# zjykzj/YOLOv4

Hardware: AMD Instinct MI355X
Metric: images/sec fwd+bwd @608x608 bs=64 per GPU (YOLOv4 training step: forward + YOLOLoss + backward) (higher is better)
Workload: dtype f32

## Files before the change

yolov4_amd/csrc/conv_planes.hip:

```cpp
#include <stdlib.h>
#include <type_traits>
#include "common.h"
#include "conv_geom.h"

namespace {

typedef _Float16 f16x8 __attribute__((ext_vector_type(8)));
typedef float f32x4v __attribute__((ext_vector_type(4)));

__device__ __host__ __forceinline__ unsigned pl_scale_exp(unsigned amax_bits) {
    const unsigned e = (amax_bits >> 23) & 0xffu;
    if (e == 0u || e == 255u) return 127u;
    int se = 268 - (int)e;
    if (se < 2) se = 2;
    if (se > 252) se = 252;
    return (unsigned)se;
}
__device__ __forceinline__ float pl_scale(const unsigned* amax) { return __uint_as_float(pl_scale_exp(amax ? *amax : 0u) << 23); }
__device__ __forceinline__ float pl_unscale(const unsigned* amax) { return __uint_as_float((254u - pl_scale_exp(amax ? *amax : 0u)) << 23); }

struct PlaneConvGeom {
    const unsigned char* src;
    const unsigned char* wt;
    float* dst; long long ldd;
    const float* res; long long ldr;
    float* stats;
    int dst_bf16;
    int cls_ntaps, cls_ph, cls_pw, Hfull, Wfull;
    int cls_dh[4], cls_dw[4], cls_slot[4];
    int B, Hs, Ws, Cs, Hd, Wd, N, k, stride, pad, M, K;
    int mtiles, ntiles;
    unsigned long long src_total_bytes;
    unsigned wt_bytes;
    const unsigned* src_amax; const unsigned* wt_amax;
};

constexpr int PROW = 128;

typedef __bf16 bf16x8 __attribute__((ext_vector_type(8)));
template <bool BF>
__device__ __forceinline__ f32x4v pl_mma(const f16x8 a, const f16x8 b, const f32x4v c) {
    if constexpr (BF) return __builtin_amdgcn_mfma_f32_16x16x32_bf16(__builtin_bit_cast(bf16x8, a), __builtin_bit_cast(bf16x8, b), c, 0, 0, 0);
    else return __builtin_amdgcn_mfma_f32_16x16x32_f16(a, b, c, 0, 0, 0);
}

#ifndef PL_ST_POL
#define PL_ST_POL 2
#endif
template <int BM, int BN, int WM, int WN, bool BF, bool YB = false, bool DG2 = false>
__global__ __launch_bounds__(WM * WN * 64, WM * WN == 8 ? 1 : 2) void conv_planes_mfma(const PlaneConvGeom g) {
    constexpr int NWAVE = WM * WN, NTHR = NWAVE * 64;
    static_assert(NWAVE == 8 || NWAVE == 4, "8 or 4 waves");
    constexpr int WTM = BM / WM, WTN = BN / WN, TM = WTM / 16, TN = WTN / 16;
    constexpr int A_BYTES = BM * PROW, B_BYTES = BN * PROW, STAGE = A_BYTES + B_BYTES;
    constexpr int NSTAGE = (NWAVE == 8 && 3 * STAGE <= 160 * 1024) ? 3 : 2;
    constexpr int KSH = BF ? 6 : 5;
    constexpr unsigned WEB = BF ? 2u : 4u;
    constexpr int PA = BM / 8 / NWAVE, PB = BN / 8 / NWAVE, NDMA = PA + PB;
    static_assert(PA >= 1 && PB >= 1 && ((NSTAGE == 3 && NDMA == 6) || (NSTAGE == 2 && NDMA == 8)),
                  "the counted vmcnt below assumes 6 (three stages) or 8 (two stages) pieces per wave and K-tile");
    typedef float accv __attribute__((ext_vector_type(4)));
    extern __shared__ __attribute__((aligned(1024))) unsigned char smem[];

    const int tid = threadIdx.x, lane = tid & 63;
    const int wave = __builtin_amdgcn_readfirstlane(tid >> 6);
    const int wm = wave / WN, wn = wave % WN;
    const int lt = y4_xcd_remap(blockIdx.x, g.mtiles * g.ntiles);
    const int mt = lt / g.ntiles, nt = lt - mt * g.ntiles;
    const int n0 = nt * BN;
    const int CC = g.Cs >> KSH;
    const int KT = (DG2 ? g.cls_ntaps : g.k * g.k) * CC;

    const int pix_per_img = g.Hd * g.Wd;
    const int b_first = (int)(((long long)mt * BM) / pix_per_img);
    const unsigned pitch = (unsigned)g.Cs * 4u;
    const unsigned long long img_bytes = (unsigned long long)g.Hs * g.Ws * pitch;
    const unsigned long long skip = (unsigned long long)b_first * img_bytes;
    const unsigned long long left = g.src_total_bytes > skip ? g.src_total_bytes - skip : 0ull;
    const __amdgpu_buffer_rsrc_t src_rsrc = y4_make_rsrc(g.src + skip, (unsigned)(left < 0xfffffff0ull ? left : 0xfffffff0ull));
    const __amdgpu_buffer_rsrc_t wt_rsrc = y4_make_rsrc(g.wt, g.wt_bytes);
    const unsigned OOB = 0xffffffffu;

    const int lr = lane >> 3, pos = lane & 7;
    unsigned a_base[PA], a_valid[PA], a_voff[PA];
#pragma unroll
    for (int i = 0; i < PA; ++i) {
        const int row = (wave * PA + i) * 8 + lr;
        const int m = mt * BM + row;
        const bool ok = m < g.M;
        const int mm = ok ? m : 0;
        const int b = mm / pix_per_img;
        const int rem = mm - b * pix_per_img;
        const int hd = rem / g.Wd, wd = rem - hd * g.Wd;
        const int hc = DG2 ? hd : hd * g.stride - g.pad, wc = DG2 ? wd : wd * g.stride - g.pad;
        const int chunk = pos ^ ((row >> 1) & 7);
        a_base[i] = (unsigned)(((b - b_first) * g.Hs + hc) * g.Ws + wc) * pitch + (unsigned)chunk * 16u;
        unsigned v = 0u;
        if constexpr (DG2) {
            for (int t = 0; t < g.cls_ntaps; ++t)
                if (ok && hc + g.cls_dh[t] < g.Hs && wc + g.cls_dw[t] < g.Ws) v |= 1u << t;
        } else {
            for (int r = 0; r < g.k; ++r)
                for (int q = 0; q < g.k; ++q)
                    if (ok && (unsigned)(hc + r) < (unsigned)g.Hs && (unsigned)(wc + q) < (unsigned)g.Ws) v |= 1u << (r * g.k + q);
        }
        a_valid[i] = v;
    }
    unsigned b_off[PB];
#pragma unroll
    for (int j = 0; j < PB; ++j) {
        const int row = (wave * PB + j) * 8 + lr;
        const int chunk = pos ^ ((row >> 1) & 7);
        b_off[j] = (n0 + row) < g.N ? (unsigned)(n0 + row) * (unsigned)g.K * WEB + (unsigned)chunk * 16u : OOB;
    }
    int ld_tap = 0, ld_r = 0, ld_q = 0, ld_cc = 0;
    int ld_slot = DG2 ? g.cls_slot[0] : 0;
    auto tap_setup = [&]() {
        unsigned toff;
        if constexpr (DG2) {
            const int t = ld_tap < g.cls_ntaps ? ld_tap : 0;
            toff = (unsigned)(g.cls_dh[t] * g.Ws + g.cls_dw[t]) * pitch;
            ld_slot = g.cls_slot[t];
        } else {
            toff = (unsigned)(ld_r * g.Ws + ld_q) * pitch;
            ld_slot = ld_tap;
        }
#pragma unroll
        for (int i = 0; i < PA; ++i) a_voff[i] = ((a_valid[i] >> ld_tap) & 1u) ? a_base[i] + toff : OOB;
    };
    tap_setup();
    typedef __attribute__((address_space(3))) void* lds_ptr;
    auto issue = [&](int stage, auto P0, auto P1) {
        constexpr int p0 = decltype(P0)::value, p1 = decltype(P1)::value;
        unsigned char* st = smem + stage * STAGE;
        const unsigned soff_a = (unsigned)ld_cc * 128u;
        const unsigned soff_b = (unsigned)(ld_slot * CC + ld_cc) * 128u;
#pragma unroll
        for (int p = p0; p < p1; ++p) {
            if (p < PA)
                __builtin_amdgcn_raw_ptr_buffer_load_lds(src_rsrc, (lds_ptr)(st + (wave * PA + p) * 1024), 16, (int)a_voff[p], (int)soff_a, 0, 0);
            else
                __builtin_amdgcn_raw_ptr_buffer_load_lds(wt_rsrc, (lds_ptr)(st + A_BYTES + (wave * PB + (p - PA)) * 1024), 16,
                                                         (int)b_off[p - PA], (int)soff_b, 0, 0);
        }
        if constexpr (p1 == NDMA) {
            if (++ld_cc == CC) {
                ld_cc = 0; ++ld_tap;
                if (++ld_q == g.k) { ld_q = 0; ++ld_r; }
                tap_setup();
            }
        }
    };
    using I0 = std::integral_constant<int, 0>; using I2 = std::integral_constant<int, 2>; using I4 = std::integral_constant<int, 4>;
    using I6 = std::integral_constant<int, NDMA>;

    accv acc0[TM][TN], acc1[BF ? 1 : TM][BF ? 1 : TN];
#pragma unroll
    for (int i = 0; i < TM; ++i)
#pragma unroll
        for (int j = 0; j < TN; ++j)
#pragma unroll
            for (int e = 0; e < 4; ++e) {
                acc0[i][j][e] = 0.f;
                if constexpr (!BF) acc1[i][j][e] = 0.f;
            }

    const int fr = lane & 15, kq = lane >> 4;
    const int sw = (fr >> 1) & 7;
    const int a_hi = (wm * WTM + fr) * PROW + ((kq ^ sw) << 4), a_lo = (wm * WTM + fr) * PROW + (((4 + kq) ^ sw) << 4);
    const int b_hi = A_BYTES + (wn * WTN + fr) * PROW + ((kq ^ sw) << 4), b_lo = A_BYTES + (wn * WTN + fr) * PROW + (((4 + kq) ^ sw) << 4);

    bool pend = false;
    auto step = [&](auto SC, const int kt) {
        constexpr int S = decltype(SC)::value;
        const unsigned char* base = smem + S * STAGE;
        f16x8 fb[TN][2];
#pragma unroll
        for (int j = 0; j < TN; ++j) {
            fb[j][0] = *reinterpret_cast<const f16x8*>(base + b_hi + j * 16 * PROW);
            fb[j][1] = *reinterpret_cast<const f16x8*>(base + b_lo + j * 16 * PROW);
        }
        f16x8 fap[2][2];
        fap[0][0] = *reinterpret_cast<const f16x8*>(base + a_hi);
        fap[0][1] = *reinterpret_cast<const f16x8*>(base + a_lo);
#pragma unroll
        for (int i = 0; i < TM; ++i) {
            if (i + 1 < TM) {
                fap[(i + 1) & 1][0] = *reinterpret_cast<const f16x8*>(base + a_hi + (i + 1) * 16 * PROW);
                fap[(i + 1) & 1][1] = *reinterpret_cast<const f16x8*>(base + a_lo + (i + 1) * 16 * PROW);
            }
            const f16x8 fa0 = fap[i & 1][0], fa1 = fap[i & 1][1];
            if (i == TM - 1) {
                __builtin_amdgcn_sched_barrier(0);
                asm volatile("s_waitcnt lgkmcnt(0)" ::: "memory");
                if (kt + 1 < KT) {
                    if constexpr (NSTAGE == 3) {
                        if (kt + 2 < KT) asm volatile("s_waitcnt vmcnt(6)" ::: "memory");
                        else asm volatile("s_waitcnt vmcnt(0)" ::: "memory");
                        __builtin_amdgcn_s_barrier();
                        if (kt + 3 < KT) { issue(S, I0{}, I2{}); pend = true; }
                    } else {
                        asm volatile("s_waitcnt vmcnt(0)" ::: "memory");
                        __builtin_amdgcn_s_barrier();
                        if (kt + 2 < KT) issue(S, I0{}, I6{});
                    }
                }
            }
            if constexpr (BF) {
#pragma unroll
                for (int j = 0; j < TN; ++j) acc0[i][j] = pl_mma<true>(fa0, fb[j][0], acc0[i][j]);
#pragma unroll
                for (int j = 0; j < TN; ++j) acc0[i][j] = pl_mma<true>(fa1, fb[j][1], acc0[i][j]);
            } else {
#pragma unroll
                for (int j = 0; j < TN; ++j) {
                    acc1[i][j] = pl_mma<false>(fa1, fb[j][0], acc1[i][j]);
                    acc1[i][j] = pl_mma<false>(fa0, fb[j][1], acc1[i][j]);
                    acc0[i][j] = pl_mma<false>(fa0, fb[j][0], acc0[i][j]);
                }
            }
            if constexpr (NSTAGE == 3) {
                if (i == 0 && pend) issue((S + 2) % NSTAGE, I2{}, I4{});
                if (i == 1 && pend) { issue((S + 2) % NSTAGE, I4{}, I6{}); pend = false; }
            }
        }
    };
    static_assert(TM >= 3, "the DMA pieces are spread over the first three row tiles");

    for (int t = 0; t < NSTAGE && t < KT; ++t) issue(t, I0{}, I6{});
    if constexpr (NSTAGE == 3) {
        if (KT >= 3) asm volatile("s_waitcnt vmcnt(12)" ::: "memory");
        else if (KT == 2) asm volatile("s_waitcnt vmcnt(6)" ::: "memory");
        else asm volatile("s_waitcnt vmcnt(0)" ::: "memory");
    } else {
        if (KT >= 2) asm volatile("s_waitcnt vmcnt(8)" ::: "memory");
        else asm volatile("s_waitcnt vmcnt(0)" ::: "memory");
    }
    __builtin_amdgcn_s_barrier();
    if constexpr (NSTAGE == 3) {
        int kt = 0;
        for (; kt + 3 <= KT; kt += 3) {
            step(std::integral_constant<int, 0>{}, kt);
            step(std::integral_constant<int, 1>{}, kt + 1);
            step(std::integral_constant<int, 2>{}, kt + 2);
        }
        if (kt < KT) step(std::integral_constant<int, 0>{}, kt);
        if (kt + 1 < KT) step(std::integral_constant<int, 1>{}, kt + 1);
    } else {
        int kt = 0;
        for (; kt + 2 <= KT; kt += 2) {
            step(std::integral_constant<int, 0>{}, kt);
            step(std::integral_constant<int, 1>{}, kt + 1);
        }
        if (kt < KT) step(std::integral_constant<int, 0>{}, kt);
    }

    const float un = BF ? 1.0f : pl_unscale(g.src_amax) * pl_unscale(g.wt_amax);
    const float un1 = un * (1.0f / 2048.0f);
    auto result = [&](int i, int j, int e) -> float {
        if constexpr (BF) return acc0[i][j][e];
        else return acc0[i][j][e] * un + acc1[i][j][e] * un1;
    };
    {
        const unsigned drow = (unsigned)g.ldd * 4u, rrow = (unsigned)g.ldr * 4u;
        const long long row0 = (long long)mt * BM;
        const unsigned long long left = (unsigned long long)(g.M - row0);
        const unsigned long long dby = left * drow, rby = g.ldr ? left * rrow : (unsigned long long)g.N * 4ull;
        const __amdgpu_buffer_rsrc_t drs = y4_make_rsrc(reinterpret_cast<char*>(g.dst) + row0 * (long long)drow, (unsigned)(dby < 0xfffffff0ull ? dby : 0xfffffff0ull));
        const __amdgpu_buffer_rsrc_t rrs = y4_make_rsrc(g.res ? reinterpret_cast<const char*>(g.res) + row0 * (long long)rrow : nullptr,
                                                        g.res ? (unsigned)(rby < 0xfffffff0ull ? rby : 0xfffffff0ull) : 0u);
        int lane_e = lane;
        asm volatile("" : "+v"(lane_e));
        const int fr = lane_e & 15, kq = lane_e >> 4;
        const int colb = n0 + wn * WTN + fr;
        const bool allc = n0 + BN <= g.N;
        if constexpr (DG2) {
            const __amdgpu_buffer_rsrc_t xrs = y4_make_rsrc(g.dst, (unsigned)((unsigned long long)g.B * g.Hfull * g.Wfull * drow));
#pragma unroll
            for (int i = 0; i < TM; ++i) {
                const int m0 = mt * BM + wm * WTM + 16 * i + 4 * kq;
                int b = m0 / pix_per_img;
                const int rem = m0 - b * pix_per_img;
                int hc = rem / g.Wd, wc = rem - hc * g.Wd;
#pragma unroll
                for (int e = 0; e < 4; ++e) {
                    const bool rok = m0 + e < g.M;
                    const unsigned po = (unsigned)((b * g.Hfull + 2 * hc + g.cls_ph) * g.Wfull + 2 * wc + g.cls_pw) * drow + (unsigned)colb * 4u;
#pragma unroll
                    for (int j = 0; j < TN; ++j) {
// ... 46 lines not shown
                        const bool cok = allc || colb + 16 * j < g.N;
                        __builtin_amdgcn_raw_buffer_store_b32(__builtin_bit_cast(unsigned, v), drs, (int)(cok ? dvo + 64u * j : 0xffffffffu), (int)(e * drow), PL_ST_POL);
                    }
            }
        }
        } else {
            float csum[TN], cssum[TN];
#pragma unroll
            for (int j = 0; j < TN; ++j) { csum[j] = 0.f; cssum[j] = 0.f; }
#pragma unroll
            for (int i = 0; i < TM; ++i) {
                const unsigned rl = (unsigned)(wm * WTM + 16 * i + 4 * kq);
                const unsigned dvo = rl * drow + (unsigned)colb * 2u;
#pragma unroll
                for (int e = 0; e < 4; ++e)
#pragma unroll
                    for (int j = 0; j < TN; ++j) {
                        const float v = result(i, j, e);
                        unsigned u = __builtin_bit_cast(unsigned, v);
                        u = (u + 0x7fffu + ((u >> 16) & 1u)) & 0xffff0000u;
                        const float vr = __builtin_bit_cast(float, u);
                        csum[j] += vr; cssum[j] += vr * vr;
                        const unsigned nb = (unsigned)__builtin_amdgcn_update_dpp(0, (int)u, 0xB1, 0xf, 0xf, true);
                        const bool cok = (allc || colb + 16 * j < g.N) && !(fr & 1);
                        __builtin_amdgcn_raw_buffer_store_b32((u >> 16) | nb, drs, (int)(cok ? dvo + 32u * j : 0xffffffffu), (int)(e * drow), PL_ST_POL);
                    }
                __builtin_amdgcn_sched_barrier(0);
            }
#pragma unroll
            for (int j = 0; j < TN; ++j) { acc0[0][j][0] = csum[j]; acc0[0][j][1] = cssum[j]; }
        }
    }
    if (g.stats) {
        __syncthreads();
        float* red = reinterpret_cast<float*>(smem);
#pragma unroll
        for (int j = 0; j < TN; ++j) {
            float cs = 0.f, css = 0.f;
            if constexpr (YB) {
                cs = acc0[0][j][0]; css = acc0[0][j][1];
            } else {
#pragma unroll
                for (int i = 0; i < TM; ++i)
#pragma unroll
                    for (int e = 0; e < 4; ++e) { const float v = acc0[i][j][e]; cs += v; css += v * v; }
            }
            cs += __shfl_xor(cs, 16, 64); css += __shfl_xor(css, 16, 64);
            cs += __shfl_xor(cs, 32, 64); css += __shfl_xor(css, 32, 64);
            if (kq == 0) {
                const int c = wn * WTN + j * 16 + fr;
                red[(wm * BN + c) * 2 + 0] = cs;
                red[(wm * BN + c) * 2 + 1] = css;
            }
        }
        __syncthreads();
        for (int c = tid; c < BN; c += NTHR) {
            float cs = 0.f, css = 0.f;
#pragma unroll
            for (int w = 0; w < WM; ++w) { cs += red[(w * BN + c) * 2]; css += red[(w * BN + c) * 2 + 1]; }
            const int n = n0 + c;
            if (n < g.N) {
                g.stats[((long long)mt * 2 + 0) * g.N + n] = cs;
                g.stats[((long long)mt * 2 + 1) * g.N + n] = css;
            }
        }
    }
}

struct PlaneWgradGeom {
    const unsigned char* x;
    const unsigned char* dy;
    float* out;
    int B, H, W, Cin, Cout, k, pad, M, J;
    int ldy_ch;
    int ntn, ntj, splits, steps_per_split;
    unsigned long long x_total_bytes, dy_total_bytes;
    const unsigned* x_amax; const unsigned* dy_amax;
};

typedef __fp16 trh4 __attribute__((__vector_size__(4 * sizeof(__fp16))));
__device__ __forceinline__ f16x8 tr_frag(const unsigned char* p) {
    typedef __attribute__((address_space(3))) trh4* lp;
    const trh4 a = __builtin_amdgcn_ds_read_tr16_b64_v4f16((lp)(p));
    const trh4 b = __builtin_amdgcn_ds_read_tr16_b64_v4f16((lp)(p + 4 * PROW));
    f16x8 r;
#pragma unroll
    for (int e = 0; e < 4; ++e) { r[e] = (_Float16)a[e]; r[4 + e] = (_Float16)b[e]; }
    return r;
}

template <int N> __device__ __forceinline__ void pl_wait_vm() {
    static_assert(N == 0 || N == 3 || N == 4 || N == 6 || N == 8 || N == 12, "add the literal");
    if constexpr (N == 0) asm volatile("s_waitcnt vmcnt(0)" ::: "memory");
    else if constexpr (N == 3) asm volatile("s_waitcnt vmcnt(3)" ::: "memory");
    else if constexpr (N == 4) asm volatile("s_waitcnt vmcnt(4)" ::: "memory");
    else if constexpr (N == 6) asm volatile("s_waitcnt vmcnt(6)" ::: "memory");
    else if constexpr (N == 8) asm volatile("s_waitcnt vmcnt(8)" ::: "memory");
    else asm volatile("s_waitcnt vmcnt(12)" ::: "memory");
}
// ... 464 lines not shown
        for (long long i = i0; i < n; i += step) {
            const int nn = (int)(i % Cout);
            const long long t = i / Cout;
            const int tp = (int)(t % kk);
            const int tap = mirror ? kk - 1 - tp : tp;
            const int c = (int)(t / kk);
            tr[i] = pl_bf16_bits(w[((long long)nn * kk + tap) * Cin + c]);
        }
}
int bf16_filter(const float* w, unsigned short* fwd, unsigned short* tr, int Cout, int Cin, int kk, bool mirror, hipStream_t st) {
    const long long n = (long long)Cout * kk * Cin;
    const int blocks = (int)((n + 255) / 256 > 2048 ? 2048 : (n + 255) / 256);
    hipLaunchKernelGGL(bf16_filter_kernel, dim3(blocks > 0 ? blocks : 1), dim3(256), 0, st, w, fwd, tr, Cout, Cin, kk, mirror ? 1 : 0);
    Y4_CHECK_LAUNCH();
    return Y4_OK;
}

template <int BM, int BN, int WM, int WN, bool BF, bool YB = false, bool DG2 = false>
int launch_conv_planes(const PlaneConvGeom& g0, hipStream_t st) {
    PlaneConvGeom g = g0;
    g.mtiles = (g.M + BM - 1) / BM;
    g.ntiles = (g.N + BN - 1) / BN;
    constexpr int NW = WM * WN;
    constexpr size_t stage = (size_t)(BM + BN) * PROW;
    constexpr size_t smem = ((NW == 8 && 3 * stage <= 160 * 1024) ? 3ull : 2ull) * stage;
    static_assert(NW == 8 || 2 * smem <= 160 * 1024, "two blocks per CU");
    static_assert(smem <= 160 * 1024, "LDS");
    auto kern = conv_planes_mfma<BM, BN, WM, WN, BF, YB, DG2>;
    static Y4DynLds lds_attr;
    if (!lds_attr.ensure(reinterpret_cast<const void*>(kern), smem)) return Y4_ERR_LAUNCH;
    y4::note_kernel("conv_planes_mfma<%d, %d, %d, %d, %s, %s, %s>", BM, BN, WM, WN, BF ? "true" : "false", YB ? "true" : "false",
                    DG2 ? "true" : "false");
    hipLaunchKernelGGL(kern, dim3(g.mtiles * g.ntiles), dim3(NW * 64), smem, st, g);
    Y4_CHECK_LAUNCH();
    return Y4_OK;
}

}

namespace y4 {

bool planes_conv_ok(int Cin, int Cout, int k, int stride) {
    return Cin > 0 && (Cin & 31) == 0 && Cout > 0 && (Cout & 3) == 0 && (k == 1 || k == 3) && (stride == 1 || stride == 2);
}

static bool conv_window_ok(int B, int Hs, int Ws, int Cs, int N, int k, int stride, bool bf) {
    const int pad = (k - 1) / 2;
    const long long Hd = (Hs + 2 * pad - k) / stride + 1, Wd = (Ws + 2 * pad - k) / stride + 1;
    if (Hd <= 0 || Wd <= 0 || (long long)B * Hd * Wd >= (1ll << 31)) return false;
    const unsigned long long img = (unsigned long long)Hs * Ws * (unsigned long long)Cs * 4ull;
    const unsigned long long wb = (unsigned long long)N * k * k * Cs * (bf ? 2ull : 4ull);
    const unsigned long long imgs_per_tile = 256ull / (unsigned long long)(Hd * Wd) + 2;
    return img * imgs_per_tile < 0xfffffff0ull && wb < 0xfffffff0ull;
}
static bool dgrad_s2_window_ok(int B, int H, int W, int Cin, int Cout, long long lddx) {
    if ((H & 1) || (W & 1)) return false;
    return conv_window_ok(B, H / 2, W / 2, Cout, Cin, 3, 1, false) &&
           (unsigned long long)B * H * W * (unsigned long long)lddx * 4ull < 0xfffffff0ull;
}
static bool wgrad_window_ok(int B, int H, int W, int Cin, int Cout, int k, int stride, bool bf) {
    const long long M = (long long)B * H * W;
    if (M >= (1ll << 31) - 65536) return false;
    if ((unsigned long long)Cout * k * k * Cin * 4ull >= 0xfffffff0ull) return false;
    int ntn, ntj, splits, sps;
    planes_wgrad_plan(B, H, W, Cin, Cout, k, &ntn, &ntj, &splits, &sps, planes_wgrad_tn(Cout, bf), bf);
    const int pad = (k - 1) / 2;
// ... 33 lines not shown
    g.src_total_bytes = (unsigned long long)B * img;
    g.wt_bytes = (unsigned)wb;
    g.src_amax = src_amax; g.wt_amax = wt_amax;
    static const int small_mode = getenv("Y4_PLANES_SMALL") ? atoi(getenv("Y4_PLANES_SMALL")) : 1;
    bool quant = false;
    {
        const long long nt = (N + 127) / 128;
        const long long b256 = (long long)((g.M + 255) / 256) * nt, b128 = (long long)((g.M + 127) / 128) * nt;
        const long long c256 = ((b256 + 255) / 256) * 2;
        const long long tail = b128 % 512;
        const long long c128 = (b128 / 512) * 2 + (tail == 0 ? 0 : (tail <= 256 ? 1 : 2));
        quant = (double)c128 * 1.08 < (double)c256;
    }
    const bool small = small_mode == 2 || (small_mode == 1 && (g.K <= 256 || quant)) || (small_mode == 4 && g.K <= 256);
    if (bf && stream_bf16_ok(g, dst_bf16)) {
        g.K = Cs;
        return dst_bf16 ? dispatch_stream_bf16<true>(g, st, nparts) : dispatch_stream_bf16<false>(g, st, nparts);
    }
    if (bf) {
        const char* bt = getenv("Y4_BF_TILE");
        const int bf_tile = bt ? atoi(bt) : 0;
        const long long mt = (g.M + 255) / 256;
        const long long r256 = (mt * ((N + 255) / 256) + 255) / 256, r128 = (mt * ((N + 127) / 128) + 255) / 256;
        const bool big = bf_tile == 2 || (bf_tile == 0 && N > 128 && (double)r256 * 2.0 <= (double)r128 * 1.25);
        if (small && !big) {
            if (nparts) *nparts = (g.M + 127) / 128;
            return dst_bf16 ? launch_conv_planes<128, 128, 2, 2, true, true>(g, st) : launch_conv_planes<128, 128, 2, 2, true>(g, st);
        }
        if (nparts) *nparts = (g.M + 255) / 256;
        if (dst_bf16) return big ? launch_conv_planes<256, 256, 2, 4, true, true>(g, st) : launch_conv_planes<256, 128, 4, 2, true, true>(g, st);
        return big ? launch_conv_planes<256, 256, 2, 4, true>(g, st) : launch_conv_planes<256, 128, 4, 2, true>(g, st);
    }
    if (dst_bf16) return Y4_ERR_SHAPE;
    if (nparts) *nparts = small ? (g.M + 127) / 128 : (g.M + 255) / 256;
    return small ? launch_conv_planes<128, 128, 2, 2, false>(g, st) : launch_conv_planes<256, 128, 4, 2, false>(g, st);
}

int planes_dgrad_s2(const void* dy, const unsigned* dy_amax, const void* wt_planes, const unsigned* wt_amax, float* dx, long long lddx,
                    int B, int H, int W, int Cin, int Cout, hipStream_t st, bool bf) {
    if ((H & 1) || (W & 1) || (Cout & 31) || (Cin & 3) || (bf && (Cout & 63))) return Y4_ERR_SHAPE;
    const int Ho = H / 2, Wo = W / 2;
    PlaneConvGeom g{};
    g.src = static_cast<const unsigned char*>(dy); g.wt = static_cast<const unsigned char*>(wt_planes);
    g.dst = dx; g.ldd = lddx;
    g.B = B; g.Hs = Ho; g.Ws = Wo; g.Cs = Cout; g.N = Cin; g.k = 3; g.stride = 1; g.pad = 0;
    g.Hd = Ho; g.Wd = Wo; g.Hfull = H; g.Wfull = W;
    if (B <= 0 || Ho <= 0 || Wo <= 0 || !dgrad_s2_window_ok(B, H, W, Cin, Cout, lddx)) return Y4_ERR_SHAPE;
    const long long M = (long long)B * Ho * Wo;
    g.M = (int)M; g.K = 9 * Cout;
    const unsigned long long img = (unsigned long long)Ho * Wo * (unsigned long long)Cout * 4ull;
    const unsigned long long wb = (unsigned long long)Cin * g.K * (bf ? 2ull : 4ull);
    g.src_total_bytes = (unsigned long long)B * img;
    g.wt_bytes = (unsigned)wb;
    g.src_amax = dy_amax; g.wt_amax = wt_amax;
    for (int c = 3; c >= 0; --c) {
        const int ph = c >> 1, pw = c & 1;
        g.cls_ph = ph; g.cls_pw = pw; g.cls_ntaps = 0;
        for (int r = 0; r < 3; ++r)
            for (int q = 0; q < 3; ++q) {
                if (((ph + 1 - r) & 1) || ((pw + 1 - q) & 1)) continue;
                const int t = g.cls_ntaps++;
                g.cls_dh[t] = (ph + 1 - r) / 2; g.cls_dw[t] = (pw + 1 - q) / 2; g.cls_slot[t] = r * 3 + q;
            }
        const int rc = bf ? launch_conv_planes<256, 128, 4, 2, true, false, true>(g, st)
                          : launch_conv_planes<256, 128, 4, 2, false, false, true>(g, st);
        if (rc != Y4_OK) return rc;
// ... 249 lines not shown
```

Baseline: 444.0.

## Add sliding-window 3x3 stride-1 conv kernel reusing input rows across taps

Adds a new fp16 planes conv kernel for 3x3 stride-1 pad-1 convolutions. It loads a contiguous window of input pixels (tile rows plus two image rows of halo) into an LDS ring once per channel chunk and serves all nine taps from that window with shifted addresses, instead of reloading the A tile for each tap. Weights are streamed per tap through a three-slot ring. The epilogue is factored into a shared helper. The window kernel becomes the default for fitting shapes, with an env var to fall back. It trades much less global/DMA traffic for more complex LDS addressing and tighter LDS limits.

```diff
diff --git a/yolov4_amd/csrc/conv_planes.hip b/yolov4_amd/csrc/conv_planes.hip
--- a/yolov4_amd/csrc/conv_planes.hip
+++ b/yolov4_amd/csrc/conv_planes.hip
@@ -47,214 +47,12 @@
 #ifndef PL_ST_POL
 #define PL_ST_POL 2
 #endif
-template <int BM, int BN, int WM, int WN, bool BF, bool YB = false, bool DG2 = false>
-__global__ __launch_bounds__(WM * WN * 64, WM * WN == 8 ? 1 : 2) void conv_planes_mfma(const PlaneConvGeom g) {
-    constexpr int NWAVE = WM * WN, NTHR = NWAVE * 64;
-    static_assert(NWAVE == 8 || NWAVE == 4, "8 or 4 waves");
+template <int BM, int BN, int WM, int WN, bool BF, bool YB, bool DG2, typename Acc0, typename Acc1>
+__device__ __forceinline__ void pl_epilogue(const PlaneConvGeom& g, Acc0& acc0, Acc1& acc1, const int mt, const int n0, const int wm,
+                                            const int wn, const int lane, const int tid, unsigned char* smem) {
+    constexpr int NTHR = WM * WN * 64;
     constexpr int WTM = BM / WM, WTN = BN / WN, TM = WTM / 16, TN = WTN / 16;
-    constexpr int A_BYTES = BM * PROW, B_BYTES = BN * PROW, STAGE = A_BYTES + B_BYTES;
-    constexpr int NSTAGE = (NWAVE == 8 && 3 * STAGE <= 160 * 1024) ? 3 : 2;
-    constexpr int KSH = BF ? 6 : 5;
-    constexpr unsigned WEB = BF ? 2u : 4u;
-    constexpr int PA = BM / 8 / NWAVE, PB = BN / 8 / NWAVE, NDMA = PA + PB;
-    static_assert(PA >= 1 && PB >= 1 && ((NSTAGE == 3 && NDMA == 6) || (NSTAGE == 2 && NDMA == 8)),
-                  "the counted vmcnt below assumes 6 (three stages) or 8 (two stages) pieces per wave and K-tile");
-    typedef float accv __attribute__((ext_vector_type(4)));
-    extern __shared__ __attribute__((aligned(1024))) unsigned char smem[];
-
-    const int tid = threadIdx.x, lane = tid & 63;
-    const int wave = __builtin_amdgcn_readfirstlane(tid >> 6);
-    const int wm = wave / WN, wn = wave % WN;
-    const int lt = y4_xcd_remap(blockIdx.x, g.mtiles * g.ntiles);
-    const int mt = lt / g.ntiles, nt = lt - mt * g.ntiles;
-    const int n0 = nt * BN;
-    const int CC = g.Cs >> KSH;
-    const int KT = (DG2 ? g.cls_ntaps : g.k * g.k) * CC;
-
     const int pix_per_img = g.Hd * g.Wd;
-    const int b_first = (int)(((long long)mt * BM) / pix_per_img);
-    const unsigned pitch = (unsigned)g.Cs * 4u;
-    const unsigned long long img_bytes = (unsigned long long)g.Hs * g.Ws * pitch;
-    const unsigned long long skip = (unsigned long long)b_first * img_bytes;
-    const unsigned long long left = g.src_total_bytes > skip ? g.src_total_bytes - skip : 0ull;
-    const __amdgpu_buffer_rsrc_t src_rsrc = y4_make_rsrc(g.src + skip, (unsigned)(left < 0xfffffff0ull ? left : 0xfffffff0ull));
-    const __amdgpu_buffer_rsrc_t wt_rsrc = y4_make_rsrc(g.wt, g.wt_bytes);
-    const unsigned OOB = 0xffffffffu;
-
-    const int lr = lane >> 3, pos = lane & 7;
-    unsigned a_base[PA], a_valid[PA], a_voff[PA];
-#pragma unroll
-    for (int i = 0; i < PA; ++i) {
-        const int row = (wave * PA + i) * 8 + lr;
-        const int m = mt * BM + row;
-        const bool ok = m < g.M;
-        const int mm = ok ? m : 0;
-        const int b = mm / pix_per_img;
-        const int rem = mm - b * pix_per_img;
-        const int hd = rem / g.Wd, wd = rem - hd * g.Wd;
-        const int hc = DG2 ? hd : hd * g.stride - g.pad, wc = DG2 ? wd : wd * g.stride - g.pad;
-        const int chunk = pos ^ ((row >> 1) & 7);
-        a_base[i] = (unsigned)(((b - b_first) * g.Hs + hc) * g.Ws + wc) * pitch + (unsigned)chunk * 16u;
-        unsigned v = 0u;
-        if constexpr (DG2) {
-            for (int t = 0; t < g.cls_ntaps; ++t)
-                if (ok && hc + g.cls_dh[t] < g.Hs && wc + g.cls_dw[t] < g.Ws) v |= 1u << t;
-        } else {
-            for (int r = 0; r < g.k; ++r)
-                for (int q = 0; q < g.k; ++q)
-                    if (ok && (unsigned)(hc + r) < (unsigned)g.Hs && (unsigned)(wc + q) < (unsigned)g.Ws) v |= 1u << (r * g.k + q);
-        }
-        a_valid[i] = v;
-    }
-    unsigned b_off[PB];
-#pragma unroll
-    for (int j = 0; j < PB; ++j) {
-        const int row = (wave * PB + j) * 8 + lr;
-        const int chunk = pos ^ ((row >> 1) & 7);
-        b_off[j] = (n0 + row) < g.N ? (unsigned)(n0 + row) * (unsigned)g.K * WEB + (unsigned)chunk * 16u : OOB;
-    }
-    int ld_tap = 0, ld_r = 0, ld_q = 0, ld_cc = 0;
-    int ld_slot = DG2 ? g.cls_slot[0] : 0;
-    auto tap_setup = [&]() {
-        unsigned toff;
-        if constexpr (DG2) {
-            const int t = ld_tap < g.cls_ntaps ? ld_tap : 0;
-            toff = (unsigned)(g.cls_dh[t] * g.Ws + g.cls_dw[t]) * pitch;
-            ld_slot = g.cls_slot[t];
-        } else {
-            toff = (unsigned)(ld_r * g.Ws + ld_q) * pitch;
-            ld_slot = ld_tap;
-        }
-#pragma unroll
-        for (int i = 0; i < PA; ++i) a_voff[i] = ((a_valid[i] >> ld_tap) & 1u) ? a_base[i] + toff : OOB;
-    };
-    tap_setup();
-    typedef __attribute__((address_space(3))) void* lds_ptr;
-    auto issue = [&](int stage, auto P0, auto P1) {
-        constexpr int p0 = decltype(P0)::value, p1 = decltype(P1)::value;
-        unsigned char* st = smem + stage * STAGE;
-        const unsigned soff_a = (unsigned)ld_cc * 128u;
-        const unsigned soff_b = (unsigned)(ld_slot * CC + ld_cc) * 128u;
-#pragma unroll
-        for (int p = p0; p < p1; ++p) {
-            if (p < PA)
-                __builtin_amdgcn_raw_ptr_buffer_load_lds(src_rsrc, (lds_ptr)(st + (wave * PA + p) * 1024), 16, (int)a_voff[p], (int)soff_a, 0, 0);
-            else
-                __builtin_amdgcn_raw_ptr_buffer_load_lds(wt_rsrc, (lds_ptr)(st + A_BYTES + (wave * PB + (p - PA)) * 1024), 16,
-                                                         (int)b_off[p - PA], (int)soff_b, 0, 0);
-        }
-        if constexpr (p1 == NDMA) {
-            if (++ld_cc == CC) {
-                ld_cc = 0; ++ld_tap;
-                if (++ld_q == g.k) { ld_q = 0; ++ld_r; }
-                tap_setup();
-            }
-        }
-    };
-    using I0 = std::integral_constant<int, 0>; using I2 = std::integral_constant<int, 2>; using I4 = std::integral_constant<int, 4>;
-    using I6 = std::integral_constant<int, NDMA>;
-
-    accv acc0[TM][TN], acc1[BF ? 1 : TM][BF ? 1 : TN];
-#pragma unroll
-    for (int i = 0; i < TM; ++i)
-#pragma unroll
-        for (int j = 0; j < TN; ++j)
-#pragma unroll
-            for (int e = 0; e < 4; ++e) {
-                acc0[i][j][e] = 0.f;
-                if constexpr (!BF) acc1[i][j][e] = 0.f;
-            }
-
-    const int fr = lane & 15, kq = lane >> 4;
-    const int sw = (fr >> 1) & 7;
-    const int a_hi = (wm * WTM + fr) * PROW + ((kq ^ sw) << 4), a_lo = (wm * WTM + fr) * PROW + (((4 + kq) ^ sw) << 4);
-    const int b_hi = A_BYTES + (wn * WTN + fr) * PROW + ((kq ^ sw) << 4), b_lo = A_BYTES + (wn * WTN + fr) * PROW + (((4 + kq) ^ sw) << 4);
-
-    bool pend = false;
-    auto step = [&](auto SC, const int kt) {
-        constexpr int S = decltype(SC)::value;
-        const unsigned char* base = smem + S * STAGE;
-        f16x8 fb[TN][2];
-#pragma unroll
-        for (int j = 0; j < TN; ++j) {
-            fb[j][0] = *reinterpret_cast<const f16x8*>(base + b_hi + j * 16 * PROW);
-            fb[j][1] = *reinterpret_cast<const f16x8*>(base + b_lo + j * 16 * PROW);
-        }
-        f16x8 fap[2][2];
-        fap[0][0] = *reinterpret_cast<const f16x8*>(base + a_hi);
-        fap[0][1] = *reinterpret_cast<const f16x8*>(base + a_lo);
-#pragma unroll
-        for (int i = 0; i < TM; ++i) {
-            if (i + 1 < TM) {
-                fap[(i + 1) & 1][0] = *reinterpret_cast<const f16x8*>(base + a_hi + (i + 1) * 16 * PROW);
-                fap[(i + 1) & 1][1] = *reinterpret_cast<const f16x8*>(base + a_lo + (i + 1) * 16 * PROW);
-            }
-            const f16x8 fa0 = fap[i & 1][0], fa1 = fap[i & 1][1];
-            if (i == TM - 1) {
-                __builtin_amdgcn_sched_barrier(0);
-                asm volatile("s_waitcnt lgkmcnt(0)" ::: "memory");
-                if (kt + 1 < KT) {
-                    if constexpr (NSTAGE == 3) {
-                        if (kt + 2 < KT) asm volatile("s_waitcnt vmcnt(6)" ::: "memory");
-                        else asm volatile("s_waitcnt vmcnt(0)" ::: "memory");
-                        __builtin_amdgcn_s_barrier();
-                        if (kt + 3 < KT) { issue(S, I0{}, I2{}); pend = true; }
-                    } else {
-                        asm volatile("s_waitcnt vmcnt(0)" ::: "memory");
-                        __builtin_amdgcn_s_barrier();
-                        if (kt + 2 < KT) issue(S, I0{}, I6{});
-                    }
-                }
-            }
-            if constexpr (BF) {
-#pragma unroll
-                for (int j = 0; j < TN; ++j) acc0[i][j] = pl_mma<true>(fa0, fb[j][0], acc0[i][j]);
-#pragma unroll
-                for (int j = 0; j < TN; ++j) acc0[i][j] = pl_mma<true>(fa1, fb[j][1], acc0[i][j]);
-            } else {
-#pragma unroll
-                for (int j = 0; j < TN; ++j) {
-                    acc1[i][j] = pl_mma<false>(fa1, fb[j][0], acc1[i][j]);
-                    acc1[i][j] = pl_mma<false>(fa0, fb[j][1], acc1[i][j]);
-                    acc0[i][j] = pl_mma<false>(fa0, fb[j][0], acc0[i][j]);
-                }
-            }
-            if constexpr (NSTAGE == 3) {
-                if (i == 0 && pend) issue((S + 2) % NSTAGE, I2{}, I4{});
-                if (i == 1 && pend) { issue((S + 2) % NSTAGE, I4{}, I6{}); pend = false; }
-            }
-        }
-    };
-    static_assert(TM >= 3, "the DMA pieces are spread over the first three row tiles");
-
-    for (int t = 0; t < NSTAGE && t < KT; ++t) issue(t, I0{}, I6{});
-    if constexpr (NSTAGE == 3) {
-        if (KT >= 3) asm volatile("s_waitcnt vmcnt(12)" ::: "memory");
-        else if (KT == 2) asm volatile("s_waitcnt vmcnt(6)" ::: "memory");
-        else asm volatile("s_waitcnt vmcnt(0)" ::: "memory");
-    } else {
-        if (KT >= 2) asm volatile("s_waitcnt vmcnt(8)" ::: "memory");
-        else asm volatile("s_waitcnt vmcnt(0)" ::: "memory");
-    }
-    __builtin_amdgcn_s_barrier();
-    if constexpr (NSTAGE == 3) {
-        int kt = 0;
-        for (; kt + 3 <= KT; kt += 3) {
-            step(std::integral_constant<int, 0>{}, kt);
-            step(std::integral_constant<int, 1>{}, kt + 1);
-            step(std::integral_constant<int, 2>{}, kt + 2);
-        }
-        if (kt < KT) step(std::integral_constant<int, 0>{}, kt);
-        if (kt + 1 < KT) step(std::integral_constant<int, 1>{}, kt + 1);
-    } else {
-        int kt = 0;
-        for (; kt + 2 <= KT; kt += 2) {
-            step(std::integral_constant<int, 0>{}, kt);
-            step(std::integral_constant<int, 1>{}, kt + 1);
-        }
-        if (kt < KT) step(std::integral_constant<int, 0>{}, kt);
-    }
-
     const float un = BF ? 1.0f : pl_unscale(g.src_amax) * pl_unscale(g.wt_amax);
     const float un1 = un * (1.0f / 2048.0f);
     auto result = [&](int i, int j, int e) -> float {
@@ -367,6 +165,7 @@
         }
     }
     if (g.stats) {
+        const int fr = lane & 15, kq = lane >> 4;
         __syncthreads();
         float* red = reinterpret_cast<float*>(smem);
 #pragma unroll
@@ -400,6 +199,397 @@
             }
         }
     }
+}
+
+template <int BM, int BN, int WM, int WN, bool BF, bool YB = false, bool DG2 = false>
+__global__ __launch_bounds__(WM * WN * 64, WM * WN == 8 ? 1 : 2) void conv_planes_mfma(const PlaneConvGeom g) {
+    constexpr int NWAVE = WM * WN;
+    static_assert(NWAVE == 8 || NWAVE == 4, "8 or 4 waves");
+    constexpr int WTM = BM / WM, WTN = BN / WN, TM = WTM / 16, TN = WTN / 16;
+    constexpr int A_BYTES = BM * PROW, B_BYTES = BN * PROW, STAGE = A_BYTES + B_BYTES;
+    constexpr int NSTAGE = (NWAVE == 8 && 3 * STAGE <= 160 * 1024) ? 3 : 2;
+    constexpr int KSH = BF ? 6 : 5;
+    constexpr unsigned WEB = BF ? 2u : 4u;
+    constexpr int PA = BM / 8 / NWAVE, PB = BN / 8 / NWAVE, NDMA = PA + PB;
+    static_assert(PA >= 1 && PB >= 1 && ((NSTAGE == 3 && NDMA == 6) || (NSTAGE == 2 && NDMA == 8)),
+                  "the counted vmcnt below assumes 6 (three stages) or 8 (two stages) pieces per wave and K-tile");
+    typedef float accv __attribute__((ext_vector_type(4)));
+    extern __shared__ __attribute__((aligned(1024))) unsigned char smem[];
+
+    const int tid = threadIdx.x, lane = tid & 63;
+    const int wave = __builtin_amdgcn_readfirstlane(tid >> 6);
+    const int wm = wave / WN, wn = wave % WN;
+    const int lt = y4_xcd_remap(blockIdx.x, g.mtiles * g.ntiles);
+    const int mt = lt / g.ntiles, nt = lt - mt * g.ntiles;
+    const int n0 = nt * BN;
+    const int CC = g.Cs >> KSH;
+    const int KT = (DG2 ? g.cls_ntaps : g.k * g.k) * CC;
+
+    const int pix_per_img = g.Hd * g.Wd;
+    const int b_first = (int)(((long long)mt * BM) / pix_per_img);
+    const unsigned pitch = (unsigned)g.Cs * 4u;
+    const unsigned long long img_bytes = (unsigned long long)g.Hs * g.Ws * pitch;
+    const unsigned long long skip = (unsigned long long)b_first * img_bytes;
+    const unsigned long long left = g.src_total_bytes > skip ? g.src_total_bytes - skip : 0ull;
+    const __amdgpu_buffer_rsrc_t src_rsrc = y4_make_rsrc(g.src + skip, (unsigned)(left < 0xfffffff0ull ? left : 0xfffffff0ull));
+    const __amdgpu_buffer_rsrc_t wt_rsrc = y4_make_rsrc(g.wt, g.wt_bytes);
+    const unsigned OOB = 0xffffffffu;
+
+    const int lr = lane >> 3, pos = lane & 7;
+    unsigned a_base[PA], a_valid[PA], a_voff[PA];
+#pragma unroll
+    for (int i = 0; i < PA; ++i) {
+        const int row = (wave * PA + i) * 8 + lr;
+        const int m = mt * BM + row;
+        const bool ok = m < g.M;
+        const int mm = ok ? m : 0;
+        const int b = mm / pix_per_img;
+        const int rem = mm - b * pix_per_img;
+        const int hd = rem / g.Wd, wd = rem - hd * g.Wd;
+        const int hc = DG2 ? hd : hd * g.stride - g.pad, wc = DG2 ? wd : wd * g.stride - g.pad;
+        const int chunk = pos ^ ((row >> 1) & 7);
+        a_base[i] = (unsigned)(((b - b_first) * g.Hs + hc) * g.Ws + wc) * pitch + (unsigned)chunk * 16u;
+        unsigned v = 0u;
+        if constexpr (DG2) {
+            for (int t = 0; t < g.cls_ntaps; ++t)
+                if (ok && hc + g.cls_dh[t] < g.Hs && wc + g.cls_dw[t] < g.Ws) v |= 1u << t;
+        } else {
+            for (int r = 0; r < g.k; ++r)
+                for (int q = 0; q < g.k; ++q)
+                    if (ok && (unsigned)(hc + r) < (unsigned)g.Hs && (unsigned)(wc + q) < (unsigned)g.Ws) v |= 1u << (r * g.k + q);
+        }
+        a_valid[i] = v;
+    }
+    unsigned b_off[PB];
+#pragma unroll
+    for (int j = 0; j < PB; ++j) {
+        const int row = (wave * PB + j) * 8 + lr;
+        const int chunk = pos ^ ((row >> 1) & 7);
+        b_off[j] = (n0 + row) < g.N ? (unsigned)(n0 + row) * (unsigned)g.K * WEB + (unsigned)chunk * 16u : OOB;
+    }
+    int ld_tap = 0, ld_r = 0, ld_q = 0, ld_cc = 0;
+    int ld_slot = DG2 ? g.cls_slot[0] : 0;
+    auto tap_setup = [&]() {
+        unsigned toff;
+        if constexpr (DG2) {
+            const int t = ld_tap < g.cls_ntaps ? ld_tap : 0;
+            toff = (unsigned)(g.cls_dh[t] * g.Ws + g.cls_dw[t]) * pitch;
+            ld_slot = g.cls_slot[t];
+        } else {
+            toff = (unsigned)(ld_r * g.Ws + ld_q) * pitch;
+            ld_slot = ld_tap;
+        }
+#pragma unroll
+        for (int i = 0; i < PA; ++i) a_voff[i] = ((a_valid[i] >> ld_tap) & 1u) ? a_base[i] + toff : OOB;
+    };
+    tap_setup();
+    typedef __attribute__((address_space(3))) void* lds_ptr;
+    auto issue = [&](int stage, auto P0, auto P1) {
+        constexpr int p0 = decltype(P0)::value, p1 = decltype(P1)::value;
+        unsigned char* st = smem + stage * STAGE;
+        const unsigned soff_a = (unsigned)ld_cc * 128u;
+        const unsigned soff_b = (unsigned)(ld_slot * CC + ld_cc) * 128u;
+#pragma unroll
+        for (int p = p0; p < p1; ++p) {
+            if (p < PA)
+                __builtin_amdgcn_raw_ptr_buffer_load_lds(src_rsrc, (lds_ptr)(st + (wave * PA + p) * 1024), 16, (int)a_voff[p], (int)soff_a, 0, 0);
+            else
+                __builtin_amdgcn_raw_ptr_buffer_load_lds(wt_rsrc, (lds_ptr)(st + A_BYTES + (wave * PB + (p - PA)) * 1024), 16,
+                                                         (int)b_off[p - PA], (int)soff_b, 0, 0);
+        }
+        if constexpr (p1 == NDMA) {
+            if (++ld_cc == CC) {
+                ld_cc = 0; ++ld_tap;
+                if (++ld_q == g.k) { ld_q = 0; ++ld_r; }
+                tap_setup();
+            }
+        }
+    };
+    using I0 = std::integral_constant<int, 0>; using I2 = std::integral_constant<int, 2>; using I4 = std::integral_constant<int, 4>;
+    using I6 = std::integral_constant<int, NDMA>;
+
+    accv acc0[TM][TN], acc1[BF ? 1 : TM][BF ? 1 : TN];
+#pragma unroll
+    for (int i = 0; i < TM; ++i)
+#pragma unroll
+        for (int j = 0; j < TN; ++j)
+#pragma unroll
+            for (int e = 0; e < 4; ++e) {
+                acc0[i][j][e] = 0.f;
+                if constexpr (!BF) acc1[i][j][e] = 0.f;
+            }
+
+    const int fr = lane & 15, kq = lane >> 4;
+    const int sw = (fr >> 1) & 7;
+    const int a_hi = (wm * WTM + fr) * PROW + ((kq ^ sw) << 4), a_lo = (wm * WTM + fr) * PROW + (((4 + kq) ^ sw) << 4);
+    const int b_hi = A_BYTES + (wn * WTN + fr) * PROW + ((kq ^ sw) << 4), b_lo = A_BYTES + (wn * WTN + fr) * PROW + (((4 + kq) ^ sw) << 4);
+
+    bool pend = false;
+    auto step = [&](auto SC, const int kt) {
+        constexpr int S = decltype(SC)::value;
+        const unsigned char* base = smem + S * STAGE;
+        f16x8 fb[TN][2];
+#pragma unroll
+        for (int j = 0; j < TN; ++j) {
+            fb[j][0] = *reinterpret_cast<const f16x8*>(base + b_hi + j * 16 * PROW);
+            fb[j][1] = *reinterpret_cast<const f16x8*>(base + b_lo + j * 16 * PROW);
+        }
+        f16x8 fap[2][2];
+        fap[0][0] = *reinterpret_cast<const f16x8*>(base + a_hi);
+        fap[0][1] = *reinterpret_cast<const f16x8*>(base + a_lo);
+#pragma unroll
+        for (int i = 0; i < TM; ++i) {
+            if (i + 1 < TM) {
+                fap[(i + 1) & 1][0] = *reinterpret_cast<const f16x8*>(base + a_hi + (i + 1) * 16 * PROW);
+                fap[(i + 1) & 1][1] = *reinterpret_cast<const f16x8*>(base + a_lo + (i + 1) * 16 * PROW);
+            }
+            const f16x8 fa0 = fap[i & 1][0], fa1 = fap[i & 1][1];
+            if (i == TM - 1) {
+                __builtin_amdgcn_sched_barrier(0);
+                asm volatile("s_waitcnt lgkmcnt(0)" ::: "memory");
+                if (kt + 1 < KT) {
+                    if constexpr (NSTAGE == 3) {
+                        if (kt + 2 < KT) asm volatile("s_waitcnt vmcnt(6)" ::: "memory");
+                        else asm volatile("s_waitcnt vmcnt(0)" ::: "memory");
+                        __builtin_amdgcn_s_barrier();
+                        if (kt + 3 < KT) { issue(S, I0{}, I2{}); pend = true; }
+                    } else {
+                        asm volatile("s_waitcnt vmcnt(0)" ::: "memory");
+                        __builtin_amdgcn_s_barrier();
+                        if (kt + 2 < KT) issue(S, I0{}, I6{});
+                    }
+                }
+            }
+            if constexpr (BF) {
+#pragma unroll
+                for (int j = 0; j < TN; ++j) acc0[i][j] = pl_mma<true>(fa0, fb[j][0], acc0[i][j]);
+#pragma unroll
+                for (int j = 0; j < TN; ++j) acc0[i][j] = pl_mma<true>(fa1, fb[j][1], acc0[i][j]);
+            } else {
+#pragma unroll
+                for (int j = 0; j < TN; ++j) {
+                    acc1[i][j] = pl_mma<false>(fa1, fb[j][0], acc1[i][j]);
+                    acc1[i][j] = pl_mma<false>(fa0, fb[j][1], acc1[i][j]);
+                    acc0[i][j] = pl_mma<false>(fa0, fb[j][0], acc0[i][j]);
+                }
+            }
+            if constexpr (NSTAGE == 3) {
+                if (i == 0 && pend) issue((S + 2) % NSTAGE, I2{}, I4{});
+                if (i == 1 && pend) { issue((S + 2) % NSTAGE, I4{}, I6{}); pend = false; }
+            }
+        }
+    };
+    static_assert(TM >= 3, "the DMA pieces are spread over the first three row tiles");
+
+    for (int t = 0; t < NSTAGE && t < KT; ++t) issue(t, I0{}, I6{});
+    if constexpr (NSTAGE == 3) {
+        if (KT >= 3) asm volatile("s_waitcnt vmcnt(12)" ::: "memory");
+        else if (KT == 2) asm volatile("s_waitcnt vmcnt(6)" ::: "memory");
+        else asm volatile("s_waitcnt vmcnt(0)" ::: "memory");
+    } else {
+        if (KT >= 2) asm volatile("s_waitcnt vmcnt(8)" ::: "memory");
+        else asm volatile("s_waitcnt vmcnt(0)" ::: "memory");
+    }
+    __builtin_amdgcn_s_barrier();
+    if constexpr (NSTAGE == 3) {
+        int kt = 0;
+        for (; kt + 3 <= KT; kt += 3) {
+            step(std::integral_constant<int, 0>{}, kt);
+            step(std::integral_constant<int, 1>{}, kt + 1);
+            step(std::integral_constant<int, 2>{}, kt + 2);
+        }
+        if (kt < KT) step(std::integral_constant<int, 0>{}, kt);
+        if (kt + 1 < KT) step(std::integral_constant<int, 1>{}, kt + 1);
+    } else {
+        int kt = 0;
+        for (; kt + 2 <= KT; kt += 2) {
+            step(std::integral_constant<int, 0>{}, kt);
+            step(std::integral_constant<int, 1>{}, kt + 1);
+        }
+        if (kt < KT) step(std::integral_constant<int, 0>{}, kt);
+    }
+
+    pl_epilogue<BM, BN, WM, WN, BF, YB, DG2>(g, acc0, acc1, mt, n0, wm, wn, lane, tid, smem);
+}
+
+constexpr int WIN_MAXW = 76;
+constexpr int WIN_PIECES = (256 + 2 * WIN_MAXW + 2 + 7) / 8;
+constexpr int WIN_RING = 3 * 128 * PROW, WIN_BUF = WIN_PIECES * 1024, WIN_ZERO = WIN_RING + 2 * WIN_BUF, WIN_LDS = WIN_ZERO + 1024;
+static_assert(WIN_LDS <= 160 * 1024, "LDS");
+
+template <int N> __device__ __forceinline__ void pl_win_wait() {
+    static_assert(N >= 0 && N <= 4, "add the literal");
+    if constexpr (N == 0) asm volatile("s_waitcnt vmcnt(0)" ::: "memory");
+    else if constexpr (N == 1) asm volatile("s_waitcnt vmcnt(1)" ::: "memory");
+    else if constexpr (N == 2) asm volatile("s_waitcnt vmcnt(2)" ::: "memory");
+    else if constexpr (N == 3) asm volatile("s_waitcnt vmcnt(3)" ::: "memory");
+    else asm volatile("s_waitcnt vmcnt(4)" ::: "memory");
+}
+
+template <int NPW>
+__global__ __launch_bounds__(512, 1) void conv_planes_mfma_win(const PlaneConvGeom g) {
+    constexpr int BM = 256, BN = 128, WM = 4, WN = 2, WTM = 64, WTN = 64, TM = 4, TN = 4, PB = 2;
+    constexpr int B_BYTES = BN * PROW;
+    static_assert(NPW >= 1 && NPW <= 7, "steps 7 and 8 issue no window piece");
+    typedef float accv __attribute__((ext_vector_type(4)));
+    extern __shared__ __attribute__((aligned(1024))) unsigned char smem[];
+
+    const int tid = threadIdx.x, lane = tid & 63;
+    const int wave = __builtin_amdgcn_readfirstlane(tid >> 6);
+    const int wm = wave / WN, wn = wave % WN;
+    const int lt = y4_xcd_remap(blockIdx.x, g.mtiles * g.ntiles);
+    const int mt = lt / g.ntiles, nt = lt - mt * g.ntiles;
+    const int n0 = nt * BN, m0 = mt * BM;
+    const int CC = g.Cs >> 5, KT = 9 * CC;
+    const int W = g.Ws;
+    const int pix_per_img = g.Hs * W;
+
+    const unsigned pitch = (unsigned)g.Cs * 4u;
+    const int p_first = m0 - W - 1;
+    const int p_base = p_first > 0 ? p_first : 0;
+    const unsigned long long skip = (unsigned long long)p_base * pitch;
+    const unsigned long long left = g.src_total_bytes > skip ? g.src_total_bytes - skip : 0ull;
+    const __amdgpu_buffer_rsrc_t src_rsrc = y4_make_rsrc(g.src + skip, (unsigned)(left < 0xfffffff0ull ? left : 0xfffffff0ull));
+    const __amdgpu_buffer_rsrc_t wt_rsrc = y4_make_rsrc(g.wt, g.wt_bytes);
+    const unsigned OOB = 0xffffffffu;
+
+    const int lr = lane >> 3, pos = lane & 7;
+    const int npieces = (BM + 2 * W + 2 + 7) >> 3;
+    unsigned w_voff[NPW];
+#pragma unroll
+    for (int i = 0; i < NPW; ++i) {
+        const int p = i * 8 + wave;
+        const int row = p * 8 + lr;
+        const int gp = p_first + row;
+        const int chunk = pos ^ ((row >> 1) & 7);
+        w_voff[i] = (p < npieces && gp >= 0) ? (unsigned)(gp - p_base) * pitch + (unsigned)chunk * 16u : OOB;
+    }
+    unsigned b_off[PB];
+#pragma unroll
+    for (int j = 0; j < PB; ++j) {
+        const int row = (wave * PB + j) * 8 + lr;
+        const int chunk = pos ^ ((row >> 1) & 7);
+        b_off[j] = (n0 + row) < g.N ? (unsigned)(n0 + row) * (unsigned)g.K * 4u + (unsigned)chunk * 16u : OOB;
+    }
+    typedef __attribute__((address_space(3))) void* lds_ptr;
+    auto issue_w = [&](const int buf, const int i, const int cc) {
+        const int p = i * 8 + wave;
+        unsigned char* d = p < npieces ? smem + WIN_RING + buf * WIN_BUF + p * 1024 : smem + WIN_ZERO;
+        __builtin_amdgcn_raw_ptr_buffer_load_lds(src_rsrc, (lds_ptr)d, 16, (int)w_voff[i], (int)((unsigned)cc * 128u), 0, 0);
+    };
+    auto issue_f = [&](const int slot, const int tap, const int cc) {
+        const unsigned soff = (unsigned)(tap * CC + cc) * 128u;
+#pragma unroll
+        for (int j = 0; j < PB; ++j)
+            __builtin_amdgcn_raw_ptr_buffer_load_lds(wt_rsrc, (lds_ptr)(smem + slot * B_BYTES + (wave * PB + j) * 1024), 16, (int)b_off[j],
+                                                     (int)soff, 0, 0);
+    };
+
+    accv acc0[TM][TN], acc1[TM][TN];
+#pragma unroll
+    for (int i = 0; i < TM; ++i)
+#pragma unroll
+        for (int j = 0; j < TN; ++j)
+#pragma unroll
+            for (int e = 0; e < 4; ++e) { acc0[i][j][e] = 0.f; acc1[i][j][e] = 0.f; }
+
+    const int fr = lane & 15, kq = lane >> 4;
+    const int swb = (fr >> 1) & 7;
+    const int b_hi = (wn * WTN + fr) * PROW + ((kq ^ swb) << 4), b_lo = (wn * WTN + fr) * PROW + (((4 + kq) ^ swb) << 4);
+    const int lrow0 = wm * WTM + fr;
+    unsigned v9[TM];
+#pragma unroll
+    for (int i = 0; i < TM; ++i) {
+        const int m = m0 + lrow0 + 16 * i;
+        const bool ok = m < g.M;
+        const int rem = (ok ? m : 0) % pix_per_img;
+        const int h = rem / W, w = rem - h * W;
+        unsigned v = 0u;
+#pragma unroll
+        for (int r = 0; r < 3; ++r)
+#pragma unroll
+            for (int q = 0; q < 3; ++q)
+                if (ok && (unsigned)(h + r - 1) < (unsigned)g.Hs && (unsigned)(w + q - 1) < (unsigned)W) v |= 1u << (r * 3 + q);
+        v9[i] = v;
+    }
+
+    auto step = [&](auto TC, const int c, const bool more) {
+        constexpr int T = decltype(TC)::value, S = T % 3;
+        const int kt = c * 9 + T;
+        const unsigned char* fbase = smem + S * B_BYTES;
+        const int wbase = WIN_RING + (c & 1) * WIN_BUF;
+        int lrow = lrow0;
+        asm volatile("" : "+v"(lrow));
+        const int shift = (T / 3) * W + (T % 3);
+        auto a_addr = [&](const int i) -> int {
+            const int row = lrow + 16 * i + shift;
+            const int off = wbase + (row << 7) + ((((row >> 1) & 7) ^ kq) << 4);
+            return ((v9[i] >> T) & 1u) ? off : WIN_ZERO;
+        };
+        f16x8 fb[TN][2];
+#pragma unroll
+        for (int j = 0; j < TN; ++j) {
+            fb[j][0] = *reinterpret_cast<const f16x8*>(fbase + b_hi + j * 16 * PROW);
+            fb[j][1] = *reinterpret_cast<const f16x8*>(fbase + b_lo + j * 16 * PROW);
+        }
+        f16x8 fap[2][2];
+        {
+            const int ad = a_addr(0);
+            fap[0][0] = *reinterpret_cast<const f16x8*>(smem + ad);
+            fap[0][1] = *reinterpret_cast<const f16x8*>(smem + (ad ^ 64));
+        }
+#pragma unroll
+        for (int i = 0; i < TM; ++i) {
+            if (i + 1 < TM) {
+                const int ad = a_addr(i + 1);
+                fap[(i + 1) & 1][0] = *reinterpret_cast<const f16x8*>(smem + ad);
+                fap[(i + 1) & 1][1] = *reinterpret_cast<const f16x8*>(smem + (ad ^ 64));
+            }
+            const f16x8 fa0 = fap[i & 1][0], fa1 = fap[i & 1][1];
+            if (i == TM - 1) {
+                __builtin_amdgcn_sched_barrier(0);
+                asm volatile("s_waitcnt lgkmcnt(0)" ::: "memory");
+                if (kt + 1 < KT) {
+                    if (kt + 2 < KT) {
+                        constexpr int WC = (T >= 1 && T - 1 < NPW ? 1 : 0) + (T < NPW ? 1 : 0);
+                        if (more) pl_win_wait<2 + WC>();
+                        else pl_win_wait<2>();
+                    } else {
+                        pl_win_wait<0>();
+                    }
+                    __builtin_amdgcn_s_barrier();
+                    if (kt + 3 < KT) issue_f(S, (T + 3) % 9, c + (T + 3) / 9);
+                }
+            }
+#pragma unroll
+            for (int j = 0; j < TN; ++j) {
+                acc1[i][j] = pl_mma<false>(fa1, fb[j][0], acc1[i][j]);
+                acc1[i][j] = pl_mma<false>(fa0, fb[j][1], acc1[i][j]);
+                acc0[i][j] = pl_mma<false>(fa0, fb[j][0], acc0[i][j]);
+            }
+            if constexpr (T < NPW) {
+                if (i == 0 && more) issue_w((c + 1) & 1, T, c + 1);
+            }
+        }
+    };
+
+    if (tid < 256) reinterpret_cast<unsigned*>(smem + WIN_ZERO)[tid] = 0u;
+#pragma unroll
+    for (int i = 0; i < NPW; ++i) issue_w(0, i, 0);
+    issue_f(0, 0, 0); issue_f(1, 1, 0); issue_f(2, 2, 0);
+    pl_win_wait<4>();
+    asm volatile("s_waitcnt lgkmcnt(0)" ::: "memory");
+    __builtin_amdgcn_s_barrier();
+    for (int c = 0; c < CC; ++c) {
+        const bool more = c + 1 < CC;
+        step(std::integral_constant<int, 0>{}, c, more); step(std::integral_constant<int, 1>{}, c, more);
+        step(std::integral_constant<int, 2>{}, c, more); step(std::integral_constant<int, 3>{}, c, more);
+        step(std::integral_constant<int, 4>{}, c, more); step(std::integral_constant<int, 5>{}, c, more);
+        step(std::integral_constant<int, 6>{}, c, more); step(std::integral_constant<int, 7>{}, c, more);
+        step(std::integral_constant<int, 8>{}, c, more);
+    }
+
+    pl_epilogue<BM, BN, WM, WN, false, false, false>(g, acc0, acc1, mt, n0, wm, wn, lane, tid, smem);
 }
 
 struct PlaneWgradGeom {
@@ -930,6 +1120,20 @@
     y4::note_kernel("conv_planes_mfma<%d, %d, %d, %d, %s, %s, %s>", BM, BN, WM, WN, BF ? "true" : "false", YB ? "true" : "false",
                     DG2 ? "true" : "false");
     hipLaunchKernelGGL(kern, dim3(g.mtiles * g.ntiles), dim3(NW * 64), smem, st, g);
+    Y4_CHECK_LAUNCH();
+    return Y4_OK;
+}
+
+template <int NPW>
+int launch_conv_planes_win(const PlaneConvGeom& g0, hipStream_t st) {
+    PlaneConvGeom g = g0;
+    g.mtiles = (g.M + 255) / 256;
+    g.ntiles = (g.N + 127) / 128;
+    auto kern = conv_planes_mfma_win<NPW>;
+    static Y4DynLds lds_attr;
+    if (!lds_attr.ensure(reinterpret_cast<const void*>(kern), (size_t)WIN_LDS)) return Y4_ERR_LAUNCH;
+    y4::note_kernel("conv_planes_mfma_win<%d>", NPW);
+    hipLaunchKernelGGL(kern, dim3(g.mtiles * g.ntiles), dim3(512), (size_t)WIN_LDS, st, g);
     Y4_CHECK_LAUNCH();
     return Y4_OK;
 }
@@ -1029,6 +1233,18 @@
         return big ? launch_conv_planes<256, 256, 2, 4, true>(g, st) : launch_conv_planes<256, 128, 4, 2, true>(g, st);
     }
     if (dst_bf16) return Y4_ERR_SHAPE;
+    {
+        const char* pw = getenv("Y4_PLANES_WINDOW");
+        const int pieces = (256 + 2 * Ws + 2 + 7) / 8;
+        const bool fits = k == 3 && stride == 1 && pad == 1 && Ws <= WIN_MAXW &&
+                          (unsigned long long)(pieces * 8 + 8) * (unsigned long long)Cs * 4ull < 0xfffffff0ull;
+        const long long b256 = (long long)((g.M + 255) / 256) * ((N + 127) / 128);
+        if (fits && !(quant && b256 > 256)) {
+            if (nparts) *nparts = (g.M + 255) / 256;
+            if (pw && atoi(pw) == 0) return launch_conv_planes<256, 128, 4, 2, false>(g, st);
+            return pieces <= 40 ? launch_conv_planes_win<5>(g, st) : pieces <= 48 ? launch_conv_planes_win<6>(g, st) : launch_conv_planes_win<7>(g, st);
+        }
+    }
     if (nparts) *nparts = small ? (g.M + 127) / 128 : (g.M + 255) / 256;
     return small ? launch_conv_planes<128, 128, 2, 2, false>(g, st) : launch_conv_planes<256, 128, 4, 2, false>(g, st);
 }
```

Result: no change. 447.4, median of 6 (+0.8%).
